# iangitonga/tinyllama.cpp

Measured on AMD Instinct MI355X. Metric: decode tok/s TinyLlama-1.1B q4 ctx=2048, 1 GPU; achieved HBM GB/s vs peak, higher is better.
Workload: dtype q4 weights x q8 activations (int8 dot, f32 accumulate); 1 GPU; TinyLlama-1.1B q4 greedy single-token decode, batch 1 per GPU, steps end at n=2048 (BASELINE.json configs[3]); ctx=2048, graph=True, steps_per_graph_replay=4, kv_cache=q8 blocks (reference layout), argmax=device, parallelism=replicas x1

## Files before the change

include/gten_hip_ab.h:

```cpp
#pragma once

#ifdef __cplusplus
extern "C" {
#endif

int gten_hip_set_decode_attn_classic(int on);

#ifdef __cplusplus
}
#endif
```

tinyllama.cpp_amd/csrc/gten_decode.hip:

```cpp
#include "gten_dev.h"
#include "gten_rt.h"
#include "gten_hip_sample.h"
#include "gten_hip_ab.h"
#include "gten_hip_prefix_decode.h"

#include <cmath>
#include <vector>
#include <algorithm>

using namespace gtd;

extern __shared__ __attribute__((aligned(16))) uint8_t g_smem[];

#define DEC_CHUNK 256
#define ATT1V_VROW 68
#define ATT1V_PCOL 72
#define DEC_MAX_LANES 4
#define DEC_ATT_MAXCH 8
#define GEMVM_F16_LDS_LIMIT 65536

static int g_only_family = -1;
#define DEC_LAUNCH(tag, kernel, grid, block, smem, ...)                                        \
    do {                                                                                       \
        if (g_only_family < 0 || g_only_family == (tag)) GTR_LAUNCH(tag, kernel, grid, block, smem, __VA_ARGS__); \
    } while (0)

#define DEC_LAUNCH_HOT(tag, kernel, grid, block, smem, hw, a) \
    DEC_LAUNCH(tag, kernel, grid, block, smem, (hw).w[0], (hw).w[1], (hw).w[2], (hw).w[3], (hw).w[4], (hw).w[5], (hw).w[6], a)

struct DecStep {
    int n;
    int advance;
    int stop;
};


struct ActStage {
    float* row;
    float* red;
    ActQ8 q8;
};

__device__ __forceinline__ ActStage carve_stage(int d)
{
    ActStage s;
    s.red = (float*)g_smem;
    s.row = (float*)(g_smem + 64);
    s.q8 = actq8_carve(g_smem + 64 + (size_t)d * 4, d >> 5);
    return s;
}
static size_t stage_bytes(int d) { return 64 + (size_t)d * 4 + (size_t)(d >> 5) * 40; }

enum { PRO_EMBED = 0, PRO_RESID = 1, PRO_ATT = 2, PRO_ATTW = 3, PRO_ACTQ8 = 4 };
enum { EPI_RAW = 0, EPI_SILUMUL = 1, EPI_STAGE = 2, EPI_STAGE_FRAG = 3 };

#define WXP_PLANES 8
#include "gten_decode_wx.h"
#include "gten_decode_wide_wx.h"
#include "gten_decode_ffn.h"
#include "gten_decode_wxp.h"
#include "gten_decode_attn.h"
#include "gten_decode_attn_exact64.h"
#include "gten_decode_attn_wide.h"
#include "gten_decode_attn_hm.h"
#include "gten_decode_sample.h"


using namespace gtr;

struct gten_hip_decoder {
    gten_hip_decoder_desc d;
    std::vector<gten_hip_layer_ptrs> layers;
    DecStep* step = nullptr;
    int32_t* tokens = nullptr;
    int32_t* result = nullptr;
    int32_t* ids_stage = nullptr;
    float *qkv_raw = nullptr, *proj_raw = nullptr, *down_raw = nullptr;
    float *scores = nullptr, *stats = nullptr, *att_part = nullptr;
    uint8_t *xbuf = nullptr, *hbuf = nullptr;
    float* act_f = nullptr;
    int8_t* act_q = nullptr;
    float* act_d = nullptr;
    int* act_sum = nullptr;
    float* best_val = nullptr;
    int* best_idx = nullptr;
    int n_best = 0;
    std::vector<DecStep> slots;
    int dev_n = -1;
    std::vector<int> dev_ns;
    int only_family = -1;
    int n_seq = 1;
    const void** kv_tab = nullptr;
    std::vector<const void*> kv_real;
    std::vector<char> kv_parked;
    void* dummy_kv = nullptr;
    int8_t* stg_q = nullptr;
    float* stg_d = nullptr;
    int* stg_sum = nullptr;
    float* stg_f = nullptr;
    float* logits_m = nullptr;
    float* gu_raw = nullptr;
    int n_chunks = 0;
    hipGraph_t graph = nullptr;
    hipGraphExec_t exec = nullptr;
    hipGraph_t graph_k = nullptr;
    hipGraphExec_t exec_k = nullptr;
    hipGraph_t graph_m[1 << DEC_MAX_LANES] = {}, graph_km[1 << DEC_MAX_LANES] = {};
    hipGraphExec_t exec_m[1 << DEC_MAX_LANES] = {}, exec_km[1 << DEC_MAX_LANES] = {};
    SampleParam* samp = nullptr;
    std::vector<SampleParam> samp_host;
    int n_sampling = 0;
    hipGraph_t s_graph = nullptr, s_graph_k = nullptr, s_graph_m[1 << DEC_MAX_LANES] = {}, s_graph_km[1 << DEC_MAX_LANES] = {};
    hipGraphExec_t s_exec = nullptr, s_exec_k = nullptr, s_exec_m[1 << DEC_MAX_LANES] = {}, s_exec_km[1 << DEC_MAX_LANES] = {};
    unsigned lane_mask = 0;
    int last_run_lanes = 0;
    const float2* rope = nullptr;
    float2* rope_now = nullptr;
    bool exact = false;
    bool attn_classic = false;
    bool persist_on = false;
    struct PersistState* persist = nullptr;
    uint8_t* hm = nullptr;
    size_t hm_seq_stride = 0, hm_cache_bytes = 0, hm_chunk_bytes = 0;
    std::vector<char> hm_dirty;
    unsigned long long hm_imports = 0, hm_import_launches = 0;
    uint8_t* pfx_hm = nullptr;
    int* share_dev = nullptr;
    const void** pfx_tab = nullptr;
    DecStep* pfx_step = nullptr;
    std::vector<const void*> pfx_kv;
    int pfx_len = 0;
    char pfx_dirty = 0;
    bool pfx_stale = false;
    std::vector<int> share_rows, share_cur;
    unsigned long long pfx_imports = 0, hm_skip_imports = 0;
    unsigned long long watch_epoch = 0;
    bool watch_foreign = false;
    int lanes = 1;
    hipStream_t lane_stream[DEC_MAX_LANES] = {nullptr, nullptr, nullptr, nullptr};
    hipEvent_t lane_fork = nullptr, lane_join[DEC_MAX_LANES] = {nullptr, nullptr, nullptr, nullptr};
};

struct LaneBufs {
    int n_seq;
    DecStep* step; int32_t* tokens; int32_t* result; const SampleParam* samp;
    float *qkv_raw, *proj_raw, *down_raw, *scores, *stats, *att_part;
    uint8_t *xbuf, *hbuf;
    float* act_f; int8_t* act_q; float* act_d; int* act_sum;
    const void** kv_tab;
    int8_t* stg_q; float* stg_d; int* stg_sum; float* stg_f;
    float* logits_m; float* gu_raw; float2* rope_now;
};
static LaneBufs lane_bufs(const gten_hip_decoder* dc, int lane)
{
    const gten_hip_decoder_desc& d = dc->d;
    const size_t SL = (size_t)(dc->n_seq / dc->lanes), o = (size_t)lane * SL;
    const size_t E = (size_t)d.n_embd, F = (size_t)d.n_ffn, dh = E / d.n_heads, KV = dh * d.n_kv_heads, V = (size_t)d.n_vocab;
    const size_t planes = dc->n_seq >= 16 ? 2 : 1, H = (size_t)d.n_heads, C = (size_t)dc->n_chunks;
    LaneBufs b;
    b.n_seq = (int)SL;
    b.step = dc->step + o; b.tokens = dc->tokens + o * (d.max_ctx + 1); b.result = dc->result + o * (d.max_ctx + 2); b.samp = dc->samp + o;
    const size_t rplanes = dc->n_seq >= 16 ? (size_t)WXP_PLANES : 1;
    b.qkv_raw = dc->qkv_raw + o * rplanes * (E + 2 * KV);
    b.proj_raw = dc->proj_raw + o * rplanes * E; b.down_raw = dc->down_raw + o * rplanes * E;
    b.scores = dc->scores + o * H * d.max_ctx; b.stats = dc->stats + o * H * C * 2; b.att_part = dc->att_part + o * H * C * dh;
    b.xbuf = dc->xbuf + o * E * 4; b.hbuf = dc->hbuf + o * E * 4;
    b.act_f = dc->act_f + o * F; b.act_q = dc->act_q + o * 2 * F; b.act_d = dc->act_d + o * (F / 32); b.act_sum = dc->act_sum + o * (F / 32);
    b.kv_tab = dc->kv_tab ? dc->kv_tab + o * d.n_layers * 2 : nullptr;
    b.stg_q = dc->stg_q ? dc->stg_q + o * 2 * E : nullptr; b.stg_d = dc->stg_d ? dc->stg_d + o * (E / 32) : nullptr;
    b.stg_sum = dc->stg_sum ? dc->stg_sum + o * (E / 32) : nullptr; b.stg_f = dc->stg_f ? dc->stg_f + o * E : nullptr;
    b.logits_m = dc->logits_m ? dc->logits_m + o * V : nullptr; b.gu_raw = dc->gu_raw ? dc->gu_raw + o * planes * 2 * F : nullptr;
    b.rope_now = dc->rope_now + o * (dh / 2);
    return b;
}

static bool g_decode_exact = false;
static bool g_exact_now = false;
static bool g_lane_skip = false;
static bool g_kv_head_major = true;
#define PFX_SHARED_DEFAULT true
static bool g_pfx_shared = PFX_SHARED_DEFAULT;
struct PfxArgs { const uint8_t* k = nullptr; const int* share = nullptr; };
extern "C" int gten_hip_set_kv_head_major(int on)
{
    g_kv_head_major = on != 0;
    return 0;
}
extern "C" int gten_hip_set_decode_exact(int on)
{
    g_decode_exact = on != 0;
    return 0;
}
static bool g_attn_classic = false;
static bool g_attn_classic_now = false;
extern "C" int gten_hip_set_decode_attn_classic(int on)
{
    g_attn_classic = on != 0;
    return 0;
}

static bool attention_grouped_ok(const AttnArgs& t, int n_seq)
{
    const int grp = t.n_heads / t.n_kv;
    const int min_seq = 8;
    if (t.adtype == GTEN_F16 && n_seq < 16) return false;
    return n_seq >= min_seq && (t.adtype == GTEN_Q8 || t.adtype == GTEN_F16) && t.d_head == 64 && (grp == 8 || grp == 4 || grp == 2 || grp == 1);
}

static int grp_shift1_of(int n_heads, int n_kv)
{
    const int grp = n_heads / n_kv;
    return (grp > 0 && (grp & (grp - 1)) == 0) ? __builtin_ctz(grp) + 1 : 0;
}

static bool attention_one_pass(int d_head);

static bool grouped_mm(const AttnArgs& t, int n_seq)
{
    return n_seq >= 16 && t.adtype == GTEN_Q8 && t.d_head == 64 && !g_exact_now;
}

static bool grouped_hm_f16(const AttnArgs& t, int n_seq)
{
    return n_seq >= 16 && t.adtype == GTEN_F16 && t.d_head == 64 && t.hm_k && !g_exact_now;
}

static bool grouped_one_pass(const AttnArgs& t, int n_seq)
{
    if (grouped_mm(t, n_seq) || grouped_hm_f16(t, n_seq)) return true;
    return attention_one_pass(t.d_head) && t.adtype == GTEN_Q8 && n_seq <= 8;
}

template <int GRP, int ADT>
static int launch_attention_g(const AttnArgs& t, int n_seq, const PfxArgs& pfx)
{
    constexpr size_t NW = (ADT == GTEN_Q8) ? 17 : 32;
    const dim3 grid(n_seq, t.n_chunks, t.n_kv);
    if constexpr (ADT == GTEN_Q8) if (grouped_mm(t, n_seq) && t.hm_k) {
        const int n_cq = (t.n_chunks + HM_WAVES - 1) / HM_WAVES;
        if (pfx.k) {
            if (n_seq >= 128)
                DEC_LAUNCH(KT_DEC_ATTN_SCORE, (k_dec_attn_hm_pfx<GRP, true>), dim3(n_seq * n_cq * t.n_kv), dim3(64 * HM_WAVES), 2048, t, n_seq, n_cq, pfx.k, pfx.share);
            else
                DEC_LAUNCH(KT_DEC_ATTN_SCORE, (k_dec_attn_hm_pfx<GRP, false>), dim3(n_seq * n_cq * t.n_kv), dim3(64 * HM_WAVES), 2048, t, n_seq, n_cq, pfx.k, pfx.share);
            return 0;
        }
        if (n_seq >= 128) DEC_LAUNCH(KT_DEC_ATTN_SCORE, (k_dec_attn_hm<GRP, true>), dim3(n_seq * n_cq * t.n_kv), dim3(64 * HM_WAVES), 2048, t, n_seq, n_cq);
        else DEC_LAUNCH(KT_DEC_ATTN_SCORE, (k_dec_attn_hm<GRP, false>), dim3(n_seq * n_cq * t.n_kv), dim3(64 * HM_WAVES), 2048, t, n_seq, n_cq);
        return 0;
    }
    if constexpr (ADT == GTEN_Q8) if (grouped_mm(t, n_seq)) {
        const size_t smem = (size_t)DEC_CHUNK * 68 + 2 * 8 * 264 * 2 + 16 * 64 + 32 * 4 + 8 * 4 + (size_t)4 * (DEC_MAXGRP + 2) * 2 + 128 + 128 * 4 + 80 + 64;
        GTR_REQUIRE((n_seq * t.n_chunks) % 8 == 0, "decoder: %d sequences x %d chunks is not a multiple of 8", n_seq, t.n_chunks);
        DEC_LAUNCH(KT_DEC_ATTN_SCORE, (k_dec_attn_mm_g<GRP>), dim3(n_seq * t.n_chunks * t.n_kv), dim3(256), smem, t, n_seq);
        return 0;
    }
    if constexpr (ADT == GTEN_Q8) if (grouped_one_pass(t, n_seq)) {
        constexpr size_t GP = (GRP + 1) / 2;
        const size_t smem = (size_t)(8 * GRP + 4 * GRP + 8 + 64) * 4 + (size_t)4 * (GRP + 2) * 2 + (size_t)(GRP + 2) * 64 + 16 +
                            (ADT == GTEN_Q8 ? 0 : (size_t)(GRP + 1) * 64 * 4) + 2 * GP * DEC_CHUNK * 4 + (size_t)DEC_CHUNK * NW * 4;
        DEC_LAUNCH(KT_DEC_ATTN_SCORE, (k_dec_attn_one_g<GRP, true, ADT>), grid, dim3(256), smem, t);
        return 0;
    }
    const size_t smem1 = (size_t)(8 * GRP + 4 * GRP + 8 + 64) * 4 + (size_t)4 * (GRP + 2) * 2 + (size_t)(GRP + 2) * 64 + 64 +
                         (ADT == GTEN_Q8 ? 0 : (size_t)(GRP + 1) * 64 * 4 + 16);
    const size_t smem2 = (size_t)((GRP + 1) / 2 * 2) * DEC_CHUNK * 4 + (size_t)DEC_CHUNK * NW * 4 + (size_t)(16 + 8 * GRP) * 4;
    const bool exact = n_seq <= 8 || g_exact_now;
    if (smem2 > 64 * 1024) {
        GTR_CHECK(hipFuncSetAttribute((const void*)k_dec_attn_pv_g<GRP, true, ADT>, hipFuncAttributeMaxDynamicSharedMemorySize, (int)smem2));
        GTR_CHECK(hipFuncSetAttribute((const void*)k_dec_attn_pv_g<GRP, false, ADT>, hipFuncAttributeMaxDynamicSharedMemorySize, (int)smem2));
    }
    if constexpr (ADT == GTEN_F16) if (grouped_hm_f16(t, n_seq)) {
        const int n_cq = (t.n_chunks + HM_WAVES - 1) / HM_WAVES;
        if (pfx.k) {
            if (n_seq >= 128)
                DEC_LAUNCH(KT_DEC_ATTN_SCORE, (k_dec_attn_hm_f16_pfx<GRP, true>), dim3(n_seq * n_cq * t.n_kv), dim3(64 * HM_WAVES), 2048, t, n_seq, n_cq, pfx.k, pfx.share);
            else
                DEC_LAUNCH(KT_DEC_ATTN_SCORE, (k_dec_attn_hm_f16_pfx<GRP, false>), dim3(n_seq * n_cq * t.n_kv), dim3(64 * HM_WAVES), 2048, t, n_seq, n_cq, pfx.k, pfx.share);
            return 0;
        }
        if (n_seq >= 128) DEC_LAUNCH(KT_DEC_ATTN_SCORE, (k_dec_attn_hm_f16<GRP, true>), dim3(n_seq * n_cq * t.n_kv), dim3(64 * HM_WAVES), 2048, t, n_seq, n_cq);
        else DEC_LAUNCH(KT_DEC_ATTN_SCORE, (k_dec_attn_hm_f16<GRP, false>), dim3(n_seq * n_cq * t.n_kv), dim3(64 * HM_WAVES), 2048, t, n_seq, n_cq);
        return 0;
    }
    if (ADT == GTEN_F16 && n_seq >= 16) {
        const size_t smem_m = (size_t)(128 + 16) * 4 + 128 + 128 + 64 + 16 + (size_t)17 * 64 * 2 + 64;
        DEC_LAUNCH(KT_DEC_ATTN_SCORE, (k_dec_attn_score_gm_f16<GRP>), grid, dim3(256), smem_m, t);
    } else if (ADT == GTEN_F16) {
        AttnArgs t1 = t;
        t1.grp_shift1 = grp_shift1_of(t.n_heads, t.n_kv);
        const AttnHotWords none{{0, 0, 0, 0, 0, 0, 0}};
        const size_t smem_s = (size_t)(16 + 3 * 64 + 16) * 4 + 32 + (size_t)3 * 64 + 64;
        DEC_LAUNCH_HOT(KT_DEC_ATTN_SCORE, (k_dec_attn_score64<GTEN_F16, true>), dim3(t.n_chunks, t.n_heads, n_seq), dim3(256), smem_s, none, t1);
    } else {
        DEC_LAUNCH(KT_DEC_ATTN_SCORE, (k_dec_attn_score_g<GRP, ADT>), grid, dim3(256), smem1, t);
    }
    if (exact) DEC_LAUNCH(KT_DEC_ATTN_PV, (k_dec_attn_pv_g<GRP, true, ADT>), grid, dim3(256), smem2, t);
    else DEC_LAUNCH(KT_DEC_ATTN_PV, (k_dec_attn_pv_g<GRP, false, ADT>), grid, dim3(256), smem2, t);
    return 0;
}

static int launch_attention_grouped(const AttnArgs& t, int n_seq, const PfxArgs& pfx = PfxArgs{})
{
    if (t.adtype == GTEN_Q8) {
        switch (t.n_heads / t.n_kv) {
        case 8: return launch_attention_g<8, GTEN_Q8>(t, n_seq, pfx);
        case 4: return launch_attention_g<4, GTEN_Q8>(t, n_seq, pfx);
        case 2: return launch_attention_g<2, GTEN_Q8>(t, n_seq, pfx);
        default: return launch_attention_g<1, GTEN_Q8>(t, n_seq, pfx);
        }
    }
    switch (t.n_heads / t.n_kv) {
    case 8: return launch_attention_g<8, GTEN_F16>(t, n_seq, pfx);
    case 4: return launch_attention_g<4, GTEN_F16>(t, n_seq, pfx);
    case 2: return launch_attention_g<2, GTEN_F16>(t, n_seq, pfx);
    default: return launch_attention_g<1, GTEN_F16>(t, n_seq, pfx);
    }
}

static bool attention_one_pass(int d_head)
{
    return d_head == 64 && !g_exact_now;
}

static int launch_attention(const AttnArgs& t0, dim3 agrid, size_t smem1)
{
    AttnArgs t = t0;
    t.grp_shift1 = grp_shift1_of(t.n_heads, t.n_kv);
    if (attention_one_pass(t.d_head)) {
        const size_t nw = (t.adtype == GTEN_Q8) ? 17 : 32;
        const size_t smem = 1152 + (size_t)2 * DEC_CHUNK * 4 + (size_t)DEC_CHUNK * nw * 4;
        const unsigned long long geo = (unsigned long long)(unsigned)t.kv_pitch | ((unsigned long long)(unsigned)t.max_ctx << 32);
        const unsigned long long heads = ((unsigned long long)(unsigned)t.n_heads << 32) | ((unsigned long long)(unsigned)t.n_kv << 40) |
                                         ((unsigned long long)(unsigned)t.grp_shift1 << 48);
        const AttnHotWords hw{{(unsigned long long)(uintptr_t)t.qkv_raw, (unsigned long long)(uintptr_t)t.rope_now, (unsigned long long)(uintptr_t)t.kcache,
                               (unsigned long long)(uintptr_t)t.step, geo, (unsigned long long)(unsigned)t.n_embd | heads, (unsigned long long)(uintptr_t)t.vcache}};
        const bool multi = agrid.z > 1 || t.kv_tab != nullptr;
        const dim3 g64(agrid.y, agrid.x, agrid.z);
        if (!multi && !g_attn_classic_now) {
            const size_t smem_v = 1152 + (size_t)(4 * ATT1V_PCOL + DEC_CHUNK) * 4 + (size_t)DEC_CHUNK * ATT1V_VROW * 4;
            if (t.adtype == GTEN_Q8) {
                GTR_CHECK(hipFuncSetAttribute((const void*)k_dec_attn_one64v<GTEN_Q8>, hipFuncAttributeMaxDynamicSharedMemorySize, (int)smem_v));
                DEC_LAUNCH_HOT(KT_DEC_ATTN_SCORE, k_dec_attn_one64v<GTEN_Q8>, g64, dim3(256), smem_v, hw, t);
            } else {
                GTR_CHECK(hipFuncSetAttribute((const void*)k_dec_attn_one64v<GTEN_F16>, hipFuncAttributeMaxDynamicSharedMemorySize, (int)smem_v));
                DEC_LAUNCH_HOT(KT_DEC_ATTN_SCORE, k_dec_attn_one64v<GTEN_F16>, g64, dim3(256), smem_v, hw, t);
            }
            return 0;
        }
        if (t.adtype == GTEN_Q8) {
            if (multi) DEC_LAUNCH_HOT(KT_DEC_ATTN_SCORE, (k_dec_attn_one64<GTEN_Q8, true>), g64, dim3(256), smem, hw, t);
            else DEC_LAUNCH_HOT(KT_DEC_ATTN_SCORE, (k_dec_attn_one64<GTEN_Q8, false>), g64, dim3(256), smem, hw, t);
        } else {
            if (multi) DEC_LAUNCH_HOT(KT_DEC_ATTN_SCORE, (k_dec_attn_one64<GTEN_F16, true>), g64, dim3(256), smem, hw, t);
            else DEC_LAUNCH_HOT(KT_DEC_ATTN_SCORE, (k_dec_attn_one64<GTEN_F16, false>), g64, dim3(256), smem, hw, t);
        }
        return 0;
    }
    if (t.d_head == 64) {
        const size_t nw = (t.adtype == GTEN_Q8) ? 17 : 32;
        const size_t smem2 = (size_t)2 * DEC_CHUNK * 4 + (size_t)DEC_CHUNK * nw * 4;
        const unsigned long long geo = (unsigned long long)(unsigned)t.kv_pitch | ((unsigned long long)(unsigned)t.max_ctx << 32);
        const unsigned long long heads = ((unsigned long long)(unsigned)t.n_heads << 32) | ((unsigned long long)(unsigned)t.n_kv << 40) |
                                         ((unsigned long long)(unsigned)t.grp_shift1 << 48);
        const AttnHotWords hs{{(unsigned long long)(uintptr_t)t.qkv_raw, (unsigned long long)(uintptr_t)t.rope_now, (unsigned long long)(uintptr_t)t.kcache,
                               (unsigned long long)(uintptr_t)t.step, geo, (unsigned long long)(unsigned)t.n_embd | heads, (unsigned long long)(uintptr_t)t.scores}};
        const AttnHotWords hp{{(unsigned long long)(uintptr_t)t.scores, (unsigned long long)(uintptr_t)t.stats, (unsigned long long)(uintptr_t)t.vcache,
                               (unsigned long long)(uintptr_t)t.step, geo, (unsigned long long)(unsigned)t.n_chunks | heads, (unsigned long long)(uintptr_t)t.att_part}};
        const bool multi = agrid.z > 1 || t.kv_tab != nullptr;
        const dim3 g64(agrid.y, agrid.x, agrid.z);
#define ATT_LAUNCH2(ADT, MULTI)                                                                                                          \
        do {                                                                                                                             \
            DEC_LAUNCH_HOT(KT_DEC_ATTN_SCORE, (k_dec_attn_score64<ADT, MULTI>), g64, dim3(256), smem1, hs, t);                           \
            DEC_LAUNCH_HOT(KT_DEC_ATTN_PV, (k_dec_attn_pv64<ADT, MULTI>), g64, dim3(256), smem2, hp, t);                                 \
        } while (0)
        if (t.adtype == GTEN_Q8) { if (multi) ATT_LAUNCH2(GTEN_Q8, true); else ATT_LAUNCH2(GTEN_Q8, false); }
        else { if (multi) ATT_LAUNCH2(GTEN_F16, true); else ATT_LAUNCH2(GTEN_F16, false); }
#undef ATT_LAUNCH2
        return 0;
    }
    DEC_LAUNCH(KT_DEC_ATTN_SCORE, k_dec_attn_score, agrid, dim3(256), smem1, t);
    DEC_LAUNCH(KT_DEC_ATTN_PV, k_dec_attn_pv, agrid, dim3(256), (size_t)2 * DEC_CHUNK * 4, t);
    return 0;
}

template <int WT, int PRO>
static GemvHotWords hot_of(const Gemv8Args& a)
{
    GemvHotWords hw;
    GemvHot& h = hw.h;
    if (PRO == PRO_RESID) { h.p0 = a.res_raw; h.p1 = a.res_a; h.p2 = a.norm_w; }
    else if (PRO == PRO_EMBED) { h.p0 = a.table; h.p1 = a.tokens; h.p2 = a.norm_w; }
    else if (PRO == PRO_ATT || PRO == PRO_ATTW) {
        h.p0 = a.att_part; h.p1 = (const void*)(uintptr_t)((unsigned)a.d_head_shift | ((unsigned)a.n_chunks << 8));
        h.p2 = (PRO == PRO_ATTW) ? a.att_stats : nullptr;
    }
    else { h.p0 = (WT == GTEN_F16) ? (const void*)a.act_f : (const void*)a.act_q; h.p1 = a.act_d; h.p2 = a.act_sum; }
    h.qs0 = a.qs[0]; h.ds0 = a.ds[0]; h.d_in = a.d_in; h.rows0 = a.rows[0]; h.step = a.step;
    return hw;
}

template <int WT, int PRO>
static GemvHotWords hot_of_gemv8(const Gemv8Args& a)
{
    GemvHotWords hw = hot_of<WT, PRO>(a);
    const unsigned long long r1 = a.n_mats > 1 ? (unsigned)a.rows[1] : 0u, r2 = a.n_mats > 2 ? (unsigned)a.rows[2] : 0u;
    hw.w[4] = (unsigned long long)(uintptr_t)(a.n_mats > 1 ? a.qs[1] : nullptr);
    hw.w[5] = (unsigned long long)(unsigned)a.d_in | ((unsigned long long)(unsigned)a.rows[0] << 16) | (r1 << 32) | (r2 << 48);
    hw.w[6] = (PRO == PRO_RESID) ? (unsigned long long)(uintptr_t)(a.n_mats > 2 ? a.qs[2] : nullptr) : (unsigned long long)(uintptr_t)a.step;
    return hw;
}

template <int WT, int PRO, int NCH, int R, int NT, int NM = 0>
static int launch_gemv8(int tag, const Gemv8Args& a, int total_rows)
{
    const int rows_per_wg = (NT / 64) * R;
    const dim3 grid((total_rows + rows_per_wg - 1) / rows_per_wg), block(NT);
    for (int k = 0; k + 1 < a.n_mats; k++) GTR_REQUIRE(a.rows[k] % R == 0, "decoder: concatenated matrices must hold a multiple of %d rows", R);
    const GemvHotWords hw = hot_of_gemv8<WT, PRO>(a);
    DEC_LAUNCH_HOT(tag, (k_dec_gemv8<WT, PRO, NCH, R, EPI_RAW, NT, NM>), grid, block, stage_bytes((PRO == PRO_ACTQ8 && WT != GTEN_F16) ? 32 : a.d_in), hw, a);
    return 0;
}

template <int WT>
static int launch_gateup8(const Gemv8Args& a, int n_ffn)
{
    const dim3 grid(n_ffn / 32), block(512);
    GTR_REQUIRE(n_ffn % 32 == 0, "decoder: n_ffn %d is not a multiple of 32", n_ffn);
    const GemvHotWords hw = hot_of_gemv8<WT, PRO_RESID>(a);
    DEC_LAUNCH_HOT(KT_DEC_GEMV_GATEUP, (k_dec_gemv8<WT, PRO_RESID, (WT == GTEN_F16 ? 4 : 1), 8, EPI_SILUMUL, 512>), grid, block, stage_bytes(a.d_in), hw, a);
    return 0;
}

static void set_mat(Gemv8Args& a, int k, const void* w, int wdtype, int rows, int cols)
{
    const size_t nb = (size_t)cols / 32;
    a.qs[k] = (const uint8_t*)w;
    a.ds[k] = (wdtype == GTEN_F16) ? nullptr
                                   : (const uint16_t*)((const uint8_t*)w + (size_t)rows * nb * (wdtype == GTEN_Q4 ? 16 : 32));
    a.rows[k] = rows;
}

template <int WT>
static int enqueue_step_q8act(gten_hip_decoder* dc)
{
    const gten_hip_decoder_desc& d = dc->d;
    const int E = d.n_embd, F = d.n_ffn, dh = E / d.n_heads, KV = dh * d.n_kv_heads;
    const size_t kv_pitch = gten_hip_row_bytes(d.adtype, KV);
    constexpr bool F16W = (WT == GTEN_F16);
    constexpr int NE = F16W ? 4 : 1;
    constexpr int NF = F16W ? 11 : 3;
    constexpr int NF12 = F16W ? 12 : NF;
    const bool wideF = F > 2048, widerF = F16W && F > NF * 512;
    float* xbuf = (float*)dc->xbuf;
    float* hbuf = (float*)dc->hbuf;
    int rc;
    for (int l = 0; l < d.n_layers; l++) {
        const gten_hip_layer_ptrs& L = dc->layers[l];
        Gemv8Args a{};
        a.step = dc->step; a.d_in = E; a.n_mats = 3;
        set_mat(a, 0, L.wq, WT, E, E); set_mat(a, 1, L.wk, WT, KV, E); set_mat(a, 2, L.wv, WT, KV, E);
        a.out = dc->qkv_raw; a.norm_w = (const uint16_t*)L.attn_norm; a.x_out = xbuf;
        if (l == 0) {
            a.table = d.embed; a.rope = dc->rope; a.rope_now = dc->rope_now; a.rope_half = dh / 2; a.n_vocab = d.n_vocab; a.tokens = dc->tokens;
            rc = launch_gemv8<WT, PRO_EMBED, NE, 2, 512>(KT_DEC_GEMV_QKV, a, E + 2 * KV);
        } else {
            a.res_a = hbuf; a.res_raw = dc->down_raw;
            rc = launch_gemv8<WT, PRO_RESID, NE, 2, 512>(KT_DEC_GEMV_QKV, a, E + 2 * KV);
        }
        if (rc) return rc;
        AttnArgs t{};
        t.step = dc->step; t.qkv_raw = dc->qkv_raw; t.kcache = (uint8_t*)L.kcache; t.vcache = (uint8_t*)L.vcache;
        t.kv_pitch = kv_pitch; t.scores = dc->scores; t.stats = dc->stats; t.att_part = dc->att_part; t.rope = dc->rope; t.rope_now = dc->rope_now;
        t.adtype = d.adtype; t.n_heads = d.n_heads; t.n_kv = d.n_kv_heads; t.d_head = dh; t.max_ctx = d.max_ctx;
        t.n_chunks = dc->n_chunks; t.n_embd = E;
        const dim3 agrid(d.n_heads, dc->n_chunks);
        const size_t smem1 = (size_t)(16 + 3 * dh + 16) * 4 + 32 + (size_t)3 * dh + 64;
        if (int arc = launch_attention(t, agrid, smem1)) return arc;
        Gemv8Args o{};
        o.step = dc->step; o.d_in = E; o.n_mats = 1; set_mat(o, 0, L.wo, WT, E, E); o.out = dc->proj_raw;
        o.att_part = dc->att_part; o.d_head = dh; o.d_head_shift = __builtin_ctz(dh); o.n_chunks = dc->n_chunks;
        o.att_stats = dc->stats;
        rc = attention_one_pass(dh) ? launch_gemv8<WT, PRO_ATTW, NE, 1, 512, 1>(KT_DEC_GEMV_O, o, E)
                                    : launch_gemv8<WT, PRO_ATT, NE, 1, 512, 1>(KT_DEC_GEMV_O, o, E);
        if (rc) return rc;
        Gemv8Args gu{};
        gu.step = dc->step; gu.d_in = E; gu.n_mats = 2; set_mat(gu, 0, L.wgate, WT, F, E); set_mat(gu, 1, L.wup, WT, F, E);
        gu.res_a = xbuf; gu.res_raw = dc->proj_raw; gu.x_out = hbuf; gu.norm_w = (const uint16_t*)L.ffn_norm;
        gu.act_q = dc->act_q; gu.act_d = dc->act_d; gu.act_sum = dc->act_sum; gu.act_f = dc->act_f;
        if ((rc = launch_gateup8<WT>(gu, F))) return rc;
        Gemv8Args dn{};
        dn.step = dc->step; dn.d_in = F; dn.n_mats = 1; set_mat(dn, 0, L.wdown, WT, E, F); dn.out = dc->down_raw;
        dn.act_q = dc->act_q; dn.act_d = dc->act_d; dn.act_sum = dc->act_sum;
// ... 1802 lines not shown
```

tinyllama.cpp_amd/hipabi.py:

```python
import ctypes as C
import os

import numpy as np

from . import build as _build

I32, F16, F32, Q8, Q4 = 0, 1, 2, 3, 4


class GtenHipError(RuntimeError):
    pass


def _sig(lib, name, res, args):
    f = getattr(lib, name)
    f.restype = res
    f.argtypes = args
    return f


class DeviceBuffer:

    def __init__(self, api, nbytes):
        self.api = api
# ... 46 lines not shown

    SYMBOLS = [
        "gten_hip_device_count", "gten_hip_init", "gten_hip_last_error", "gten_hip_stream", "gten_hip_sync", "gten_hip_select_stream", "gten_hip_stream_wait", "gten_hip_stream_idle",
        "gten_hip_malloc", "gten_hip_free", "gten_hip_memset", "gten_hip_memcpy_h2d", "gten_hip_memcpy_d2h",
        "gten_hip_memcpy_d2d", "gten_hip_prof_enable", "gten_hip_prof_read", "gten_hip_prof_family_name",
        "gten_hip_selftest_q8scale", "gten_hip_row_bytes", "gten_hip_pack_weight", "gten_hip_token_embed",
        "gten_hip_block_rows", "gten_hip_set_block_rows", "gten_hip_matmul_2d", "gten_hip_rms_norm", "gten_hip_rotary_emb", "gten_hip_silu", "gten_hip_mul",
        "gten_hip_add", "gten_hip_qkv_attn", "gten_hip_argmax_row", "gten_hip_set_prefill_exact", "gten_hip_set_decode_exact", "gten_hip_set_decode_persistent", "gten_hip_persist_status", "gten_hip_set_row_segments", "gten_hip_row_segments_ok", "gten_hip_copy_ranges",
        "gten_hip_decoder_create", "gten_hip_decoder_destroy", "gten_hip_decoder_set_tokens",
        "gten_hip_decoder_step", "gten_hip_decoder_steps", "gten_hip_decoder_generate", "gten_hip_decoder_generate_multi", "gten_hip_decoder_step_ragged", "gten_hip_decoder_result", "gten_hip_decoder_time_family",
        "gten_hip_decoder_create_multi", "gten_hip_decoder_set_tokens_seq", "gten_hip_decoder_result_seq",
        "gten_hip_decoder_logits_seq",
        "gten_hip_decoder_lane_info", "gten_hip_set_lane_skip", "gten_hip_decoder_slot_start", "gten_hip_decoder_slot_start_until", "gten_hip_decoder_slot_park", "gten_hip_decoder_slot_bind", "gten_hip_decoder_slots_apply", "gten_hip_decoder_run", "gten_hip_decoder_run_lanes", "gten_hip_decoder_slot_ids", "gten_hip_decoder_slot_ids_all",
        "gten_hip_set_kv_head_major", "gten_hip_decoder_kv_info", "gten_hip_kv_watch_selftest", "gten_hip_set_ffn_streamed", "gten_hip_set_wx_planes",
    ]
    SAMPLE_SYMBOLS = ["gten_hip_decoder_set_sampling", "gten_hip_sample_rows"]
    AB_SYMBOLS = ["gten_hip_set_decode_attn_classic"]
    SCORE_SYMBOLS = ["gten_hip_row_logprobs"]
    PREFIX_SYMBOLS = ["gten_hip_block_rows_prefixed"]
    PREFIX_DECODE_SYMBOLS = ["gten_hip_decoder_prefix_set", "gten_hip_decoder_slot_share", "gten_hip_decoder_prefix_info",
                             "gten_hip_set_prefix_decode_shared"]

    def __init__(self, path=None):
        path = path or _build.HIP_LIB
        if not os.path.exists(path):
            raise GtenHipError(f"{path} is missing: run __graft_entry__.build() (hipcc --offload-arch=gfx950)")
        self.path = path
        self.lib = L = C.CDLL(path, mode=C.RTLD_GLOBAL)
        vp, sz, ci = C.c_void_p, C.c_size_t, C.c_int
        self._count = _sig(L, "gten_hip_device_count", ci, [])
        self._init = _sig(L, "gten_hip_init", ci, [ci])
        self._err = _sig(L, "gten_hip_last_error", C.c_char_p, [])
        self._stream = _sig(L, "gten_hip_stream", vp, [])
        self._sync = _sig(L, "gten_hip_sync", ci, [])
        self._selftest_q8 = _sig(L, "gten_hip_selftest_q8scale", ci, [C.POINTER(C.c_ulonglong), C.POINTER(C.c_ulonglong)])
        self._malloc = _sig(L, "gten_hip_malloc", ci, [C.POINTER(vp), sz])
        self._free = _sig(L, "gten_hip_free", ci, [vp])
        self._memset = _sig(L, "gten_hip_memset", ci, [vp, ci, sz])
        self._h2d = _sig(L, "gten_hip_memcpy_h2d", ci, [vp, vp, sz])
        self._d2h = _sig(L, "gten_hip_memcpy_d2h", ci, [vp, vp, sz])
        self._d2d = _sig(L, "gten_hip_memcpy_d2d", ci, [vp, vp, sz])
        self._row_bytes = _sig(L, "gten_hip_row_bytes", sz, [ci, ci])
        self._prof_enable = _sig(L, "gten_hip_prof_enable", ci, [ci])
        self._prof_read = _sig(L, "gten_hip_prof_read", ci, [ci, C.POINTER(ci), C.POINTER(C.c_double)])
        self._prof_name = _sig(L, "gten_hip_prof_family_name", C.c_char_p, [ci])
        self._pack = _sig(L, "gten_hip_pack_weight", ci, [vp, ci, ci, ci, vp])
        self._embed = _sig(L, "gten_hip_token_embed", ci, [vp, ci, ci, vp, vp, ci, sz, ci, ci, ci])
        self._matmul = _sig(L, "gten_hip_matmul_2d", ci, [vp, ci, sz, vp, ci, vp, ci, sz, ci, ci, ci, ci])
        self._rms = _sig(L, "gten_hip_rms_norm", ci, [vp, ci, sz, vp, vp, sz, ci, ci, ci])
        self._rope = _sig(L, "gten_hip_rotary_emb", ci, [vp, ci, sz, ci, ci, ci, ci])
        self._silu = _sig(L, "gten_hip_silu", ci, [vp, vp, ci, sz, ci, ci, ci])
        self._mul = _sig(L, "gten_hip_mul", ci, [vp, vp, vp, ci, sz, ci, ci, ci])
        self._add = _sig(L, "gten_hip_add", ci, [vp, vp, vp, ci, sz, ci, ci, ci])
        self._attn = _sig(L, "gten_hip_qkv_attn", ci, [vp, vp, vp, vp, ci, sz, sz, sz, ci, ci, ci, ci, ci])
        self._prefill_exact = _sig(L, "gten_hip_set_prefill_exact", ci, [ci])
        self._block_rows = _sig(L, "gten_hip_block_rows", ci, [C.POINTER(BlockDesc), ci, ci])
        self._block_rows_prefixed = _sig(L, "gten_hip_block_rows_prefixed", ci, [C.POINTER(BlockDesc), ci, vp, vp, ci])
        self._set_block_rows = _sig(L, "gten_hip_set_block_rows", ci, [ci])
        self._prefix_decode_shared = _sig(L, "gten_hip_set_prefix_decode_shared", ci, [ci])
        self._decode_exact = _sig(L, "gten_hip_set_decode_exact", ci, [ci])
        self._decode_attn_classic = _sig(L, "gten_hip_set_decode_attn_classic", ci, [ci])
        self._decode_persistent = _sig(L, "gten_hip_set_decode_persistent", ci, [ci])
        self._kv_head_major = _sig(L, "gten_hip_set_kv_head_major", ci, [ci])
        self._kv_watch_selftest = _sig(L, "gten_hip_kv_watch_selftest", ci, [])
        self._ffn_streamed = _sig(L, "gten_hip_set_ffn_streamed", ci, [ci])
        self._wx_planes = _sig(L, "gten_hip_set_wx_planes", ci, [ci])
        self._lane_skip = _sig(L, "gten_hip_set_lane_skip", ci, [ci])
        self._persist_status = _sig(L, "gten_hip_persist_status", ci, [C.POINTER(ci), C.POINTER(C.c_ulonglong), C.POINTER(C.c_uint), C.c_void_p, ci])
        self._set_row_segments = _sig(L, "gten_hip_set_row_segments", ci, [C.c_void_p, ci])
        self._copy_ranges = _sig(L, "gten_hip_copy_ranges", ci, [C.c_void_p, ci])
        self._set_sampling = _sig(L, "gten_hip_decoder_set_sampling", ci, [vp, ci, ci, C.c_float, C.c_uint64, C.c_uint32])
        self._sample_rows = _sig(L, "gten_hip_sample_rows", ci, [vp, ci, ci, C.c_longlong, vp, vp, C.c_uint64, vp, vp, vp])
        self._row_logprobs = _sig(L, "gten_hip_row_logprobs", ci, [vp, ci, ci, C.c_longlong, vp, vp, vp, vp])
        self._argmax_row = _sig(L, "gten_hip_argmax_row", ci, [vp, ci, vp])
        self.initialised = False

    def _check(self, rc):
        if rc != 0:
            raise GtenHipError(f"gten_hip error {rc}: {self._err().decode(errors='replace')}")

    def device_count(self):
        return self._count()

    def init(self, device=0):
        if self.device_count() <= device:
            raise GtenHipError(f"no MI355X visible (device_count={self.device_count()}, asked for {device}); "
                               "there is no CPU fallback for the gten_hip path")
        self._check(self._init(device))
        self.initialised = True
        return self

    def sync(self):
        self._check(self._sync())

    def selftest_q8scale(self):
        a, b = C.c_ulonglong(0), C.c_ulonglong(0)
        self._check(self._selftest_q8(C.byref(a), C.byref(b)))
        return a.value, b.value

    def stream(self):
        return self._stream()

    def set_row_segments(self, starts):
        if not starts:
            self._check(self._set_row_segments(None, 0))
            return
        a = np.ascontiguousarray(starts, dtype=np.int32)
        self._check(self._set_row_segments(a.ctypes.data_as(C.c_void_p), len(a) - 1))

    def copy_ranges(self, ranges):
        class R(C.Structure):
            _fields_ = [("dst", C.c_void_p), ("src", C.c_void_p), ("bytes", C.c_size_t)]
        arr = (R * len(ranges))(*[R(int(d), int(s), int(b)) for d, s, b in ranges])
        self._check(self._copy_ranges(C.cast(arr, C.c_void_p), len(ranges)))

    def sample_rows(self, logits, n_rows, n_vocab, row_stride, top_k, temp, seed, stream, position):
        def per_row(v, dt):
            a = np.ascontiguousarray(np.broadcast_to(np.asarray(v, dtype=dt), (n_rows,)))
            return a, a.ctypes.data_as(C.c_void_p)
        (k, kp), (t, tp), (s, sp), (p, pp) = (per_row(top_k, np.int32), per_row(temp, np.float32), per_row(stream, np.uint32),
                                              per_row(position, np.int32))
        out = DeviceBuffer(self, max(4 * n_rows, 4))
        self._check(self._sample_rows(logits.ptr, n_rows, n_vocab, row_stride, kp, tp, C.c_uint64(int(seed)), sp, pp, out.ptr))
        return out.download(np.int32)[:n_rows].copy()

    def sample_rows_rc(self, logits, n_rows, n_vocab, row_stride, top_k, temp, seed=0, stream=0, position=1):
        k, t = np.full(max(n_rows, 1), top_k, np.int32), np.full(max(n_rows, 1), temp, np.float32)
        s, p = np.full(max(n_rows, 1), stream, np.uint32), np.full(max(n_rows, 1), position, np.int32)
        out = DeviceBuffer(self, 4 * max(n_rows, 1))
        return self._sample_rows(logits.ptr, n_rows, n_vocab, row_stride, k.ctypes.data_as(C.c_void_p), t.ctypes.data_as(C.c_void_p),
                                 C.c_uint64(int(seed)), s.ctypes.data_as(C.c_void_p), p.ctypes.data_as(C.c_void_p), out.ptr)

    def row_logprobs(self, logits, n_rows, n_vocab, row_stride, targets):
        t = DeviceBuffer.from_numpy(self, np.ascontiguousarray(targets, dtype=np.int32))
        out = DeviceBuffer(self, 12 * n_rows)
        self._check(self._row_logprobs(logits.ptr, n_rows, n_vocab, row_stride, t.ptr, out.ptr, out.ptr + 4 * n_rows, out.ptr + 8 * n_rows))
        got = out.download(np.uint8)
        return got[: 4 * n_rows].view(np.float32).copy(), got[4 * n_rows: 8 * n_rows].view(np.int32).copy(), got[8 * n_rows:].view(np.int32).copy()

    def row_logprobs_rc(self, logits, n_rows, n_vocab, row_stride):
        buf = DeviceBuffer(self, 16 * max(n_rows, 1))
        buf.zero()
        return self._row_logprobs(logits.ptr, n_rows, n_vocab, row_stride, buf.ptr, buf.ptr + 4 * max(n_rows, 1), None, None)

    def argmax_row(self, logits, n, offset=0):
        out = DeviceBuffer(self, 4)
        self._check(self._argmax_row(logits.ptr + offset, n, out.ptr))
        return int(out.download(np.int32)[0])

    def set_decode_exact(self, on):
        self._check(self._decode_exact(1 if on else 0))

    def set_decode_attn_classic(self, on):
        self._check(self._decode_attn_classic(1 if on else 0))

    def set_prefix_decode_shared(self, on):
        self._check(self._prefix_decode_shared(-1 if on is None else 1 if on else 0))

    def set_kv_head_major(self, on):
        self._check(self._kv_head_major(1 if on else 0))

    def set_ffn_streamed(self, on):
        self._check(self._ffn_streamed(1 if on else 0))

    def set_wx_planes(self, on):
        self._check(self._wx_planes(1 if on else 0))

    def kv_watch_selftest(self):
        return int(self._kv_watch_selftest())

    def set_decode_persistent(self, on):
        self._check(self._decode_persistent(1 if on else 0))

    def set_lane_skip(self, on):
        self._check(self._lane_skip(1 if on else 0))

    def persist_status(self, n_stamps=0):
        nd, nl, ab = C.c_int(0), C.c_ulonglong(0), C.c_uint(0)
        st = (C.c_uint * max(n_stamps, 1))()
        self._check(self._persist_status(C.byref(nd), C.byref(nl), C.byref(ab), C.cast(st, C.c_void_p) if n_stamps else None, n_stamps))
        return nd.value, nl.value, ab.value, list(st)[:n_stamps]

    def set_prefill_exact(self, on):
        self._check(self._prefill_exact(1 if on else 0))

    def select_stream(self, idx):
        self._check(self.lib.gten_hip_select_stream(int(idx)))

    def set_block_rows(self, on):
        self._check(self._set_block_rows(1 if on else 0))

    def block_rows(self, n, start_pos, ints, bufs):
        d = BlockDesc()
        for k, v in ints.items():
            setattr(d, k, int(v))
        for k, v in bufs.items():
            setattr(d, k, v.ptr)
        rc = self._block_rows(C.byref(d), n, start_pos)
        if rc == 1:
            return False
        self._check(rc)
        return True

    def block_rows_prefixed(self, n, ints, bufs, k_prefix, v_prefix, prefix_len):
        d = BlockDesc()
        for k, v in ints.items():
            setattr(d, k, int(v))
        for k, v in bufs.items():
            setattr(d, k, v.ptr)
        rc = self._block_rows_prefixed(C.byref(d), n, getattr(k_prefix, "ptr", k_prefix), getattr(v_prefix, "ptr", v_prefix), int(prefix_len))
        if rc == 1:
            return False
        self._check(rc)
        return True

    def prof_enable(self, on):
        self._check(self._prof_enable(1 if on else 0))

    def prof_family_index(self, wanted):
        fam = 0
        while True:
            name = self._prof_name(fam)
            if name is None:
                raise KeyError(wanted)
            if name.decode() == wanted:
                return fam
            fam += 1

    def prof_read(self):
        out = {}
        fam = 0
        while True:
            name = self._prof_name(fam)
            if name is None:
                break
            n, ms = C.c_int(0), C.c_double(0.0)
            self._check(self._prof_read(fam, C.byref(n), C.byref(ms)))
            if n.value:
                out[name.decode()] = (n.value, ms.value)
            fam += 1
        return out

    def row_bytes(self, dtype, cols):
        return self._row_bytes(dtype, cols)

    def alloc(self, nbytes):
        return DeviceBuffer(self, nbytes)

    def upload(self, arr):
        return DeviceBuffer.from_numpy(self, arr)

    def upload_weight(self, blocks, dtype, rows, cols):
        src = self.upload(blocks)
        dst = self.alloc(src.nbytes)
        self._check(self._pack(src.ptr, dtype, rows, cols, dst.ptr))
        self.sync()
        src.free()
        return dst

    def token_embed(self, w, w_dtype, n_vocab, tokens, out, out_dtype, n, d, start_pos=0, out_pitch=None):
        self._check(self._embed(w.ptr, w_dtype, n_vocab, tokens.ptr, out.ptr, out_dtype,
                                out_pitch or self.row_bytes(out_dtype, d), n, d, start_pos))

    def matmul_2d(self, x, x_dtype, w, w_dtype, out, out_dtype, n, d_in, d_out, start_pos=0,
                  x_pitch=None, out_pitch=None):
        self._check(self._matmul(x.ptr, x_dtype, x_pitch or self.row_bytes(x_dtype, d_in), w.ptr, w_dtype,
                                 out.ptr, out_dtype, out_pitch or self.row_bytes(out_dtype, d_out),
                                 n, d_in, d_out, start_pos))

    def rms_norm(self, x, dtype, w, out, n, d, start_pos=0):
        p = self.row_bytes(dtype, d)
        self._check(self._rms(x.ptr, dtype, p, w.ptr, out.ptr, p, n, d, start_pos))

    def rotary_emb(self, x, dtype, n, d, d_head, start_pos=0):
        self._check(self._rope(x.ptr, dtype, self.row_bytes(dtype, d), n, d, d_head, start_pos))

    def silu(self, x, out, dtype, n, d, start_pos=0):
        self._check(self._silu(x.ptr, out.ptr, dtype, self.row_bytes(dtype, d), n, d, start_pos))

    def mul(self, a, b, out, dtype, n, d, start_pos=0):
        self._check(self._mul(a.ptr, b.ptr, out.ptr, dtype, self.row_bytes(dtype, d), n, d, start_pos))

    def add(self, a, b, out, dtype, n, d, start_pos=0):
        self._check(self._add(a.ptr, b.ptr, out.ptr, dtype, self.row_bytes(dtype, d), n, d, start_pos))

    def qkv_attn(self, q, k, v, out, dtype, n, n_heads, n_kv_heads, d_head, start_pos=0):
        qp = self.row_bytes(dtype, n_heads * d_head)
        kp = self.row_bytes(dtype, n_kv_heads * d_head)
        self._check(self._attn(q.ptr, k.ptr, v.ptr, out.ptr, dtype, qp, kp, qp, n, n_heads, n_kv_heads, d_head, start_pos))


_api = None


def load(device=None):
    global _api
    if _api is None:
        _api = GtenHip()
    if device is not None and not _api.initialised:
        _api.init(device)
    return _api
```

Baseline: 2103 tok/s.

## Add warp-specialized 512-thread one-pass decode attention with V-widening helper waves

Adds a new single-pass attention kernel for head dim 64 that launches 512 threads, where four extra helper waves load V rows and dequantize them into shared memory while the first four waves compute scores, the softmax max and the sum. This overlaps the V load and widening with the score and softmax phases, work the 256-thread variant did in sequence. The new kernel becomes the default non-multi path, and the old v-kernel stays reachable with mode 2. The cost is larger blocks, which may lower occupancy, and more register pressure from holding the loaded row words.

New measurement: 2129 tok/s (median of 6 runs). 1.3% higher.

```diff
diff --git a/include/gten_hip_ab.h b/include/gten_hip_ab.h
--- a/include/gten_hip_ab.h
+++ b/include/gten_hip_ab.h
@@ -4,7 +4,7 @@
 extern "C" {
 #endif
 
-int gten_hip_set_decode_attn_classic(int on);
+int gten_hip_set_decode_attn_classic(int v);
 
 #ifdef __cplusplus
 }
diff --git a/tinyllama.cpp_amd/csrc/gten_decode.hip b/tinyllama.cpp_amd/csrc/gten_decode.hip
--- a/tinyllama.cpp_amd/csrc/gten_decode.hip
+++ b/tinyllama.cpp_amd/csrc/gten_decode.hip
@@ -60,6 +60,7 @@
 #include "gten_decode_ffn.h"
 #include "gten_decode_wxp.h"
 #include "gten_decode_attn.h"
+#include "gten_decode_attn_w.h"
 #include "gten_decode_attn_exact64.h"
 #include "gten_decode_attn_wide.h"
 #include "gten_decode_attn_hm.h"
@@ -117,7 +118,7 @@
     const float2* rope = nullptr;
     float2* rope_now = nullptr;
     bool exact = false;
-    bool attn_classic = false;
+    int attn_classic = 0;
     bool persist_on = false;
     struct PersistState* persist = nullptr;
     uint8_t* hm = nullptr;
@@ -191,11 +192,12 @@
     g_decode_exact = on != 0;
     return 0;
 }
-static bool g_attn_classic = false;
-static bool g_attn_classic_now = false;
-extern "C" int gten_hip_set_decode_attn_classic(int on)
-{
-    g_attn_classic = on != 0;
+static int g_attn_classic = 0;
+static int g_attn_classic_now = 0;
+extern "C" int gten_hip_set_decode_attn_classic(int v)
+{
+    GTR_REQUIRE(v >= 0 && v <= 2, "gten_hip_set_decode_attn_classic: %d is not 0, 1 or 2", v);
+    g_attn_classic = v;
     return 0;
 }
 
@@ -337,8 +339,18 @@
                                (unsigned long long)(uintptr_t)t.step, geo, (unsigned long long)(unsigned)t.n_embd | heads, (unsigned long long)(uintptr_t)t.vcache}};
         const bool multi = agrid.z > 1 || t.kv_tab != nullptr;
         const dim3 g64(agrid.y, agrid.x, agrid.z);
-        if (!multi && !g_attn_classic_now) {
+        if (!multi && g_attn_classic_now != 1) {
             const size_t smem_v = 1152 + (size_t)(4 * ATT1V_PCOL + DEC_CHUNK) * 4 + (size_t)DEC_CHUNK * ATT1V_VROW * 4;
+            if (g_attn_classic_now == 0) {
+                if (t.adtype == GTEN_Q8) {
+                    GTR_CHECK(hipFuncSetAttribute((const void*)k_dec_attn_one64w<GTEN_Q8>, hipFuncAttributeMaxDynamicSharedMemorySize, (int)smem_v));
+                    DEC_LAUNCH_HOT(KT_DEC_ATTN_SCORE, k_dec_attn_one64w<GTEN_Q8>, g64, dim3(512), smem_v, hw, t);
+                } else {
+                    GTR_CHECK(hipFuncSetAttribute((const void*)k_dec_attn_one64w<GTEN_F16>, hipFuncAttributeMaxDynamicSharedMemorySize, (int)smem_v));
+                    DEC_LAUNCH_HOT(KT_DEC_ATTN_SCORE, k_dec_attn_one64w<GTEN_F16>, g64, dim3(512), smem_v, hw, t);
+                }
+                return 0;
+            }
             if (t.adtype == GTEN_Q8) {
                 GTR_CHECK(hipFuncSetAttribute((const void*)k_dec_attn_one64v<GTEN_Q8>, hipFuncAttributeMaxDynamicSharedMemorySize, (int)smem_v));
                 DEC_LAUNCH_HOT(KT_DEC_ATTN_SCORE, k_dec_attn_one64v<GTEN_Q8>, g64, dim3(256), smem_v, hw, t);
diff --git a/tinyllama.cpp_amd/csrc/gten_decode_attn_w.h b/tinyllama.cpp_amd/csrc/gten_decode_attn_w.h
--- /dev/null
+++ b/tinyllama.cpp_amd/csrc/gten_decode_attn_w.h
@@ -0,0 +1,211 @@
+#ifndef ATT1W_SPLIT_A
+#define ATT1W_SPLIT_A 8
+#endif
+#ifndef ATT1W_SPLIT_B
+#define ATT1W_SPLIT_B 12
+#endif
+template <int ADT>
+__global__ __launch_bounds__(512) void k_dec_attn_one64w(const unsigned long long h0, const unsigned long long h1, const unsigned long long h2,
+                                                        const unsigned long long h3, const unsigned long long h4, const unsigned long long h5,
+                                                        const unsigned long long h6, const AttnArgs a0)
+{
+    AttnArgs a = a0;
+    a.qkv_raw = from_word<float>(h0); a.rope_now = from_word<float2>(h1); a.kcache = (uint8_t*)from_word<uint8_t>(h2);
+    a.step = from_word<DecStep>(h3); a.kv_pitch = (size_t)(unsigned)(h4 & 0xffffffffull); a.max_ctx = (int)(h4 >> 32);
+    a.n_embd = (int)(unsigned)(h5 & 0xffffffffull); a.n_heads = (int)((h5 >> 32) & 0xffu); a.n_kv = (int)((h5 >> 40) & 0xffu); a.grp_shift1 = (int)(h5 >> 48);
+    a.vcache = (uint8_t*)from_word<uint8_t>(h6);
+    constexpr int dh = 64, nblk = 2;
+    constexpr int NW = (ADT == GTEN_Q8) ? 17 : 32;
+    constexpr int VS = ATT1V_VROW, PS = ATT1V_PCOL;
+    const int h = blockIdx.y, chunk = blockIdx.x, c0 = chunk * DEC_CHUNK;
+    const int grp = a.grp_shift1 ? (1 << (a.grp_shift1 - 1)) : a.n_heads / a.n_kv, g = a.grp_shift1 ? (h >> (a.grp_shift1 - 1)) : h / grp;
+    const int kv_dim = a.n_kv * dh;
+    const size_t head_bytes = (ADT == GTEN_Q8) ? (size_t)nblk * GTEN_Q8_BYTES : (size_t)dh * 2;
+
+    float* red = (float*)g_smem;
+    float* qf = red + 16 + dh;
+    float* kf = qf + dh;
+    float* qd = kf + dh;
+    float* kd = qd + 8;
+    uint16_t* d16 = (uint16_t*)(kd + 8);
+    int8_t* qi8 = (int8_t*)(d16 + 16);
+    int8_t* ki8 = qi8 + dh;
+    int8_t* vi8 = ki8 + dh;
+    float* pt = (float*)(g_smem + 1152);
+    float* part = pt + 4 * PS;
+    float* vf = part + DEC_CHUNK;
+
+    const int pw = __builtin_amdgcn_readfirstlane((int)(threadIdx.x >> 6));
+    const bool helper = pw >= 4;
+    const int lt = threadIdx.x & 255, t = threadIdx.x & 63;
+    const int c = c0 + lt;
+    const int roff = (pw == 4) ? a.n_embd + g * dh : (pw >= 5) ? a.n_embd + kv_dim + g * dh : h * dh;
+    const float raw = a.qkv_raw[roff + t];
+    const float2 rot = a.rope_now[t & 31];
+    __builtin_amdgcn_sched_barrier(0);
+    const int cs = min(c, a.max_ctx - 1);
+    const unsigned pitch_w = (unsigned)(a.kv_pitch >> 2);
+    const gmem_u32 rp = as_global((helper ? a.vcache : a.kcache) + (size_t)g * head_bytes) + (unsigned)cs * pitch_w;
+    unsigned rw[NW];
+    {
+        typedef unsigned u4u __attribute__((ext_vector_type(4), aligned(4)));
+#pragma unroll
+        for (int j = 0; j + 4 <= NW; j += 4) {
+            const u4u q = *(const __attribute__((address_space(1))) u4u*)(rp + j);
+            rw[j] = q.x; rw[j + 1] = q.y; rw[j + 2] = q.z; rw[j + 3] = q.w;
+        }
+#pragma unroll
+        for (int j = NW & ~3; j < NW; j++) rw[j] = rp[j];
+    }
+    __builtin_amdgcn_sched_barrier(0);
+    const int n = a.step->n, pos = n - 1;
+    if (c0 >= n) return;
+
+    const bool has_new = (pos >= c0) && (pos < c0 + DEC_CHUNK);
+    const bool writer = has_new && (h == g * grp);
+    float vnew = 0.f;
+    if (pw == 0 || (has_new && (pw == 4 || pw == 5))) {
+        const int r = (pw == 0) ? 0 : pw - 3;
+        int8_t* dq = (r == 0) ? qi8 : (r == 1) ? ki8 : vi8;
+        float* dd = (r == 0) ? qd : (r == 1) ? kd : kd + 4;
+        const float v = head_prep_cs(raw, true, r != 2, rot, dh, ADT, dq, dd, d16 + 4 * r);
+        if (r == 0) qf[t] = v;
+        if (r == 1) kf[t] = v;
+        if (r == 2) vnew = v;
+        if (r >= 1 && writer) {
+            uint8_t* row = ((r == 1) ? a.kcache : a.vcache) + (size_t)pos * a.kv_pitch + (size_t)g * head_bytes;
+            if (ADT == GTEN_Q8) {
+                uint8_t* blk = row + (size_t)(t >> 5) * GTEN_Q8_BYTES;
+                store_global<uint8_t>(blk + 2 + (t & 31), (uint8_t)dq[t]);
+                if ((t & 31) == 0) store_global<uint16_t>(blk, d16[4 * r + (t >> 5)]);
+            } else {
+                store_global<uint16_t>((uint16_t*)row + t, f2h(v));
+            }
+        }
+    }
+    __syncthreads();
+
+    auto widen = [&](const int j0, const int j1) {
+        if (c == pos) return;
+        const bool live = c < n;
+        float4* dst = (float4*)(vf + lt * VS);
+#pragma unroll
+        for (int j = j0; j < j1; j++) {
+            float f[4];
+#pragma unroll
+            for (int i = 0; i < 4; i++) {
+                const int e = 4 * j + i;
+                float x;
+                if (ADT == GTEN_Q8) {
+                    const int b = (e < 32) ? 2 + e : 4 + e;
+                    const int q = (int)(int8_t)(uint8_t)(rw[b >> 2] >> (8 * (b & 3)));
+                    const float d = h2f((uint16_t)((e < 32) ? (rw[0] & 0xffffu) : (rw[8] >> 16)));
+                    x = (float)q * d;
+                } else {
+                    x = h2f((uint16_t)((e & 1) ? (rw[e >> 1] >> 16) : (rw[e >> 1] & 0xffffu)));
+                }
+                f[i] = live ? x : 0.f;
+            }
+            dst[j] = make_float4(f[0], f[1], f[2], f[3]);
+        }
+    };
+
+    float sc = -INFINITY, mx = 0.f, ex = 0.f, sm = 0.f;
+    if (!helper) {
+        const float scale = 1.0f / sqrtf((float)dh);
+        float acc = 0.f;
+        if (ADT == GTEN_Q8) {
+            const int* qi = (const int*)qi8;
+            int isum = 0;
+#pragma unroll
+            for (int j = 0; j < 8; j++) isum = dot4(qi[j], (int)__builtin_amdgcn_alignbit(rw[j + 1], rw[j], 16), isum);
+            acc += (float)isum * (qd[0] * h2f((uint16_t)(rw[0] & 0xffffu)));
+            isum = 0;
+#pragma unroll
+            for (int j = 0; j < 8; j++) isum = dot4(qi[8 + j], (int)rw[9 + j], isum);
+            acc += (float)isum * (qd[1] * h2f((uint16_t)(rw[8] >> 16)));
+        } else {
+#pragma unroll
+            for (int j = 0; j < 32; j++) {
+                acc += qf[2 * j] * h2f((uint16_t)(rw[j] & 0xffffu));
+                acc += qf[2 * j + 1] * h2f((uint16_t)(rw[j] >> 16));
+            }
+        }
+        if (has_new) {
+            float accn = 0.f;
+            if (ADT == GTEN_Q8) {
+                const int* qi = (const int*)qi8;
+                const int* ki = (const int*)ki8;
+#pragma unroll
+                for (int b = 0; b < nblk; b++) {
+                    int isum = 0;
+#pragma unroll
+                    for (int j = 0; j < 8; j++) isum = dot4(qi[b * 8 + j], ki[b * 8 + j], isum);
+                    accn += (float)isum * (qd[b] * kd[b]);
+                }
+            } else {
+                for (int e = 0; e < dh; e++) accn += qf[e] * kf[e];
+            }
+            if (c == pos) acc = accn;
+        }
+        sc = (c < n) ? acc * scale : -INFINITY;
+        const float wm = wave_max_dpp(sc);
+        if (t == 0) red[pw] = wm;
+    } else {
+        widen(0, ATT1W_SPLIT_A);
+    }
+    __syncthreads();
+    if (!helper) {
+        const float4 m4 = *(const float4*)red;
+        mx = fmaxf(fmaxf(fmaxf(m4.x, m4.y), m4.z), m4.w);
+        ex = (c < n) ? expf(sc - mx) : 0.f;
+        const float ws = wave_sum(ex);
+        if (t == 0) red[4 + pw] = ws;
+    } else {
+        widen(ATT1W_SPLIT_A, ATT1W_SPLIT_B);
+    }
+    __syncthreads();
+    if (!helper) {
+        const float4 s4 = *(const float4*)(red + 4);
+        sm = 0.f;
+        sm += s4.x; sm += s4.y; sm += s4.z; sm += s4.w;
+        float pr = (c < n) ? ex / sm : 0.f;
+        if (ADT == GTEN_Q8) {
+            const Q8Scale s8 = q8_scale_from_absmax(max32(fabsf(pr)));
+            if (c < n) pr = (float)q8_round(pr, s8.scale) * s8.ddeq;
+        } else {
+            pr = h2f(f2h(pr));
+        }
+        pt[(lt & 3) * PS + (lt >> 2)] = pr;
+    } else {
+        widen(ATT1W_SPLIT_B, 16);
+        if (has_new && pw == 5) vf[(pos - c0) * VS + t] = vnew;
+    }
+    __syncthreads();
+
+    if (!helper) {
+        const int e = t, cg = pw;
+        const float* vcol = vf + cg * VS + e;
+        const float4* pc = (const float4*)(pt + cg * PS);
+        float o = 0.f;
+#pragma unroll
+        for (int j = 0; j < DEC_CHUNK / 16; j++) {
+            const float4 p4 = pc[j];
+            o = o + p4.x * vcol[(4 * j + 0) * 4 * VS];
+            o = o + p4.y * vcol[(4 * j + 1) * 4 * VS];
+            o = o + p4.z * vcol[(4 * j + 2) * 4 * VS];
+            o = o + p4.w * vcol[(4 * j + 3) * 4 * VS];
+        }
+        part[lt] = o;
+    }
+    __syncthreads();
+    if (threadIdx.x < dh) {
+        float r = 0.f;
+        for (int gi = 0; gi < 4; gi++) r += part[gi * dh + threadIdx.x];
+        a.att_part[((size_t)h * a.n_chunks + chunk) * dh + threadIdx.x] = r;
+    }
+    if (threadIdx.x == 64) {
+        a.stats[((size_t)h * a.n_chunks + chunk) * 2 + 0] = mx;
+        a.stats[((size_t)h * a.n_chunks + chunk) * 2 + 1] = sm;
+    }
+}
diff --git a/tinyllama.cpp_amd/hipabi.py b/tinyllama.cpp_amd/hipabi.py
--- a/tinyllama.cpp_amd/hipabi.py
+++ b/tinyllama.cpp_amd/hipabi.py
@@ -222,7 +222,7 @@
         self._check(self._decode_exact(1 if on else 0))
 
     def set_decode_attn_classic(self, on):
-        self._check(self._decode_attn_classic(1 if on else 0))
+        self._check(self._decode_attn_classic(int(on)))
 
     def set_prefix_decode_shared(self, on):
         self._check(self._prefix_decode_shared(-1 if on is None else 1 if on else 0))
```
